# uoguelph-mlrg/Theano-MPI

Measured on NVIDIA B200. Metric: AlexNet-128b BSP seconds per 5120 images (train+comm, device-timed, max over ranks), lower is better.
Workload: dtype bf16; 1 GPU; model=AlexNet, global_batch=128, input=3x227x227, parallelism=dp1, rule=BSP, push_master=False, cuda_graph=True, overlap=True

## Files before the change

### theanompi_b200/csrc/api.h

```cpp
#pragma once
#include <cuda_runtime.h>
#include <stdint.h>
#include "common.cuh"

namespace tmpi {

constexpr int kMaxRanks = 8;
constexpr int kMaxCommBlocks = 1024;

struct CommCtx {
  void* arena[kMaxRanks];
  uint32_t* sig[kMaxRanks];
  uint32_t* epoch;
  void* mc_arena;
  int rank, world;
  long long spin_limit;
};

struct FusedArgs {
  CommCtx ctx;
  long long w_off, g_off, u_off, h_off, wire_off;
  const uint8_t* block_group;
  GroupTable tab;
  const float* lr_ptr;
  float mu;
  int nesterov;
  float inv_k;
  long long lo, hi;
  int wire16;
  int pre_reduced;
  int push_master = 1;
};

struct ReduceArgs {
  CommCtx ctx;
  long long src_off, dst_off, h_off;
  const uint8_t* block_group;
  GroupTable tab;
  float scale;
  long long lo, hi;
  int skip_local_groups;
};

void gemm_set_debug(int flags);
void gemm_set_bulk(int mask);
void gemm_rs_configure(int world, const void* const* peer_g , const void* local_g);
void gemm_rs_add_range(const void* c_lo, const void* c_hi, long long blo, long long per);
void gemm_rs_clear();
int gemm_plan_splits(int tiles, int num_kb, int sms);
int gemm_plan_tall(long long M, int nt, int out_bf16, int sms);
void gemm_bf16(const void* A, const void* B, void* C, const float* bias, int M, int N, int K, long long lda, long long ldb,
               long long ldc, int a_mn, int b_mn, int out_bf16, int bias_mode, int relu, float alpha, int bn_hint, int splitk,
               cudaStream_t st, int tf32 = 0);

void conv_fprop_bf16(const void* x, const void* w, void* y, const float* bias, int N, int H, int W, int Ctot, int c_off, int Cg, int KH,
                     int KW, int Ho, int Wo, int S, int P, int O, long long ldc, int relu, int out_bf16, int dgrad, cudaStream_t st, int tf32 = 0);
void conv_wgrad_bf16(const void* dy, const void* x, void* dw, int N, int H, int W, int Ctot, int c_off, int Cg, int KH, int KW, int Ho,
                     int Wo, int S, int P, int O, long long ldy, cudaStream_t st, int tf32 = 0);
void conv_fprop2_bf16(const void* x, const void* w0, const void* w1, void* y0, void* y1, const float* bias0, const float* bias1, int N, int H,
                      int W, int Ctot, int c_off0, int c_off1, int Cg, int KH, int KW, int Ho, int Wo, int S, int P, int O, long long ldc,
                      int relu, int out_bf16, int dgrad, cudaStream_t st, int tf32 = 0);
void conv_wgrad2_bf16(const void* dy0, const void* dy1, const void* x, void* dw0, void* dw1, int N, int H, int W, int Ctot, int c_off0,
                      int c_off1, int Cg, int KH, int KW, int Ho, int Wo, int S, int P, int O, long long ldy, cudaStream_t st, int tf32 = 0);

void space_to_depth(const void* x, void* y, int N, int H, int W, int C, int S, int Hs, int Ws, int Cp, int P, cudaStream_t st);
void s2d_filter(const void* src, void* dst, int O, int KH, int KW, int C, int S, int KHs, int KWs, int Cp, int dir, cudaStream_t st);
void conv_weight_flip(const void* w, void* wt, int O, int KH, int KW, int Cg, cudaStream_t st);
void lrn_fwd(const void* x, void* y, long long rows, int C, int n, float k, float alpha, float beta, cudaStream_t st);
void lrn_bwd(const void* x, const void* dy, void* dx, long long rows, int C, int n, float k, float alpha, float beta, cudaStream_t st);
void pool_fwd(const void* x, void* y, void* arg, int N, int H, int W, int C, int Ho, int Wo, int k, int s, int p, int is_max, cudaStream_t st);
void pool_bwd(const void* dy, const void* arg, void* dx, int N, int H, int W, int C, int Ho, int Wo, int k, int s, int p, int is_max, cudaStream_t st);
void dropout_fwd(const void* x, void* y, void* mask, long long n, float p_drop, unsigned long long seed, int layer, const void* step, cudaStream_t st);
void dropout_bwd(const void* dy, const void* mask, void* dx, long long n, cudaStream_t st);
void advance_step(void* step, cudaStream_t st);
void softmax_xent(const void* logits, const void* labels, void* dlogits, void* rowstat, void* out3, int B, int C, float weight, cudaStream_t st);
void relu_bias_bwd(const void* dy, const void* y, void* dym, void* db, long long R, int C, long long ld, int relu, cudaStream_t st);
void relu_bias_bwd2(const void* dy, const void* y, void* dym, void* db, void* db1, int c_split, long long R, int C, long long ld, int relu,
                    cudaStream_t st);
void maxpool_relu_bias_bwd(const void* dyp, const void* arg, const void* y, void* dym, void* db0, void* db1, int c_split, int N, int H,
                           int W, int C, int Ho, int Wo, int k, int s, int p, cudaStream_t st);
void im2col(const void* x, void* col, int N, int H, int W, int Ctot, int c_off, int Cg, int KH, int KW, int Ho, int Wo, int s, int p,
            long long ldcol, cudaStream_t st);
void col2im(const void* dcol, void* dx, int N, int H, int W, int Ctot, int c_off, int Cg, int KH, int KW, int Ho, int Wo, int s, int p,
            long long ldcol, cudaStream_t st);
void pad_rows(const void* src, void* dst, long long rows, int cols, long long src_ld, long long dst_ld, cudaStream_t st);
void transpose_bf16(const void* src, void* dst, int R, int C, cudaStream_t st);
// ... 8 lines not shown
void dropout_fwd_f32(const void* x, void* y, void* mask, long long n, float p_drop, unsigned long long seed, int layer, const void* step,
                     cudaStream_t st);
void dropout_bwd_f32(const void* dy, const void* mask, void* dx, long long n, cudaStream_t st);
void softmax_xent_f32(const void* logits, const void* labels, void* dlogits, void* rowstat, void* out3, int B, int C, float weight, cudaStream_t st);
void relu_bias_bwd2_f32(const void* dy, const void* y, void* dym, void* db, void* db1, int c_split, long long R, int C, long long ld, int relu,
                        cudaStream_t st);
void bias_act_f32(const void* acc, const void* bias, void* y, int R, int C, int relu, cudaStream_t st);
void im2col_f32(const void* x, void* col, int N, int H, int W, int Ctot, int c_off, int Cg, int KH, int KW, int Ho, int Wo, int s, int p,
                long long ldcol, cudaStream_t st);
void col2im_f32(const void* dcol, void* dx, int N, int H, int W, int Ctot, int c_off, int Cg, int KH, int KW, int Ho, int Wo, int s, int p,
                long long ldcol, cudaStream_t st);
void pad_rows_f32(const void* src, void* dst, long long rows, int cols, long long src_ld, long long dst_ld, cudaStream_t st);
void space_to_depth_f32(const void* x, void* y, int N, int H, int W, int C, int S, int Hs, int Ws, int Cp, int P, cudaStream_t st);
void s2d_filter_pack_f32(const void* src, void* dst, int O, int KH, int KW, int C, int S, int KHs, int KWs, int Cp, cudaStream_t st);

void bn_forward(const void* x, const void* res, void* y, const void* gamma, const void* beta, void* mean, void* rstd, void* run_mean,
                void* run_var, void* scratch, long long R, int C, float momentum, float eps, int training, int relu, int f32, cudaStream_t st);
void bn_backward(const void* x, const void* dy, const void* y, void* dx, void* dres, const void* gamma, const void* mean, const void* rstd,
                 void* dgamma, void* dbeta, void* scratch, long long R, int C, int relu, int f32, cudaStream_t st);
void add_tensors(const void* a, const void* b, void* y, long long n, int f32, cudaStream_t st);
void add4_tensors(const void* a, const void* b, const void* c, const void* d, void* y, long long n, int f32, cudaStream_t st);

void lstm_cell_fwd(const void* gx, const void* gh, const void* c_prev, const void* h_prev, const void* mask, void* act, void* c_out, void* h_out,
                   int B, int H, int f32, cudaStream_t st);
void lstm_cell_bwd(const void* dh_out, const void* dh_rec, const void* dh_pass_in, const void* dc_next, const void* act, const void* c,
                   const void* c_prev, const void* mask, void* dG, void* dc_prev, void* dh_pass, int B, int H, int f32, cudaStream_t st);
void embedding_fwd(const void* ids, const void* W, void* out, long long n, int D, int f32, cudaStream_t st);
void embedding_bwd(const void* ids, const void* dout, void* dW, long long n, int D, long long V, int f32, cudaStream_t st);
void masked_mean_fwd(const void* h, const void* mask, void* out, int Tn, int B, int H, int f32, cudaStream_t st);
void masked_mean_bwd(const void* dout, const void* mask, void* dh, int Tn, int B, int H, int f32, cudaStream_t st);

void sgd_flat(void* W, const void* G, void* U, void* H, const void* block_group, const GroupTable& tab, const void* lr_ptr, float mu,
              int nesterov, float inv_k, long long lo, long long hi, int filter, cudaStream_t st);
void adam_flat(void* W, const void* G, void* M, void* V, void* H, const void* block_group, const GroupTable& tab, const void* lr_ptr, void* step,
               float b1, float b2, float eps, long long lo, long long hi, cudaStream_t st);
void fused_allreduce_sgd(const FusedArgs& a, int algo, int max_blocks, cudaStream_t st);
void push_master_slices(const FusedArgs& a, int max_blocks, cudaStream_t st);
void allreduce_flat(const ReduceArgs& a, int algo, int max_blocks, cudaStream_t st);
void device_barrier(const CommCtx& c, cudaStream_t st);
void easgd_elastic(void* w, void* h, void* center, float alpha, long long n, int max_blocks, int lockfree, cudaStream_t st);
void ticket_acquire(const CommCtx& c, int owner, void* local_state, cudaStream_t st);
void ticket_release(const CommCtx& c, int owner, void* local_state, cudaStream_t st);
void copy_flat(void* dst, void* dst_h, const void* src, long long n, int max_blocks, const void* gate, cudaStream_t st);
void gosgd_push(const CommCtx& c, void* state, int dest, long long w_off, long long snap_off, long long n, int max_blocks, cudaStream_t st);
void gosgd_poll_merge(const CommCtx& c, void* state, long long w_off, long long h_off, long long snap_off, long long n, int max_blocks,
                      cudaStream_t st);
void gosgd_merge(void* w, void* h, const void* b, float a_self, float a_src, long long n, int max_blocks, cudaStream_t st);
void bias_act_cast(const void* acc, const void* bias, void* y, int R, int C, int relu, cudaStream_t st);
void cast_flat(const void* src, void* dst, long long n, int kind, cudaStream_t st);
void sum_chunks(const void* src, void* dst, long long chunk, int nchunks, int is_half, cudaStream_t st);
void vecadd(void* cur, const void* tmp, long long n, int is_half, cudaStream_t st);

}
```

### theanompi_b200/csrc/binding.cpp

```cpp
#include <pybind11/pybind11.h>
#include <pybind11/stl.h>

#include <cstring>
#include <memory>
#include <vector>

#include "api.h"
#include "peer_arena.h"

namespace py = pybind11;
using namespace tmpi;
typedef uintptr_t ptr_t;

static inline void* P(ptr_t p) { return reinterpret_cast<void*>(p); }
static inline cudaStream_t S(ptr_t s) { return reinterpret_cast<cudaStream_t>(s); }
static inline cudaStream_t S_(ptr_t s) { return reinterpret_cast<cudaStream_t>(s); }

static GroupTable make_table(const std::vector<float>& lr_mult, const std::vector<float>& wd, const std::vector<int>& exch) {
  GroupTable t;
  for (int i = 0; i < kMaxGroups; ++i) {
    t.lr_mult[i] = i < (int)lr_mult.size() ? lr_mult[i] : 1.f;
    t.wd[i] = i < (int)wd.size() ? wd[i] : 0.f;
    t.exch[i] = i < (int)exch.size() ? exch[i] : 1;
  }
// ... 120 lines not shown
  m.def("pad_rows_f32", [](ptr_t src, ptr_t dst, long long rows, int cols, long long src_ld, long long dst_ld, ptr_t st) {
    pad_rows_f32(P(src), P(dst), rows, cols, src_ld, dst_ld, S(st)); });
  m.def("space_to_depth_f32", [](ptr_t x, ptr_t y, int N, int H, int W, int C, int S, int Hs, int Ws, int Cp, int Pd, ptr_t st) {
    space_to_depth_f32(P(x), P(y), N, H, W, C, S, Hs, Ws, Cp, Pd, S_(st)); });
  m.def("s2d_filter_pack_f32", [](ptr_t src, ptr_t dst, int O, int KH, int KW, int C, int S, int KHs, int KWs, int Cp, ptr_t st) {
    s2d_filter_pack_f32(P(src), P(dst), O, KH, KW, C, S, KHs, KWs, Cp, S_(st)); });

  m.def("bn_forward", [](ptr_t x, ptr_t res, ptr_t y, ptr_t gamma, ptr_t beta, ptr_t mean, ptr_t rstd, ptr_t run_mean, ptr_t run_var, ptr_t scratch,
                         long long R, int C, float momentum, float eps, int training, int relu, int f32, ptr_t st) {
    bn_forward(P(x), P(res), P(y), P(gamma), P(beta), P(mean), P(rstd), P(run_mean), P(run_var), P(scratch), R, C, momentum, eps, training, relu,
               f32, S(st)); });
  m.def("bn_backward", [](ptr_t x, ptr_t dy, ptr_t y, ptr_t dx, ptr_t dres, ptr_t gamma, ptr_t mean, ptr_t rstd, ptr_t dgamma, ptr_t dbeta,
                          ptr_t scratch, long long R, int C, int relu, int f32, ptr_t st) {
    bn_backward(P(x), P(dy), P(y), P(dx), P(dres), P(gamma), P(mean), P(rstd), P(dgamma), P(dbeta), P(scratch), R, C, relu, f32, S(st)); });
  m.def("add4_tensors", [](ptr_t a, ptr_t b, ptr_t c, ptr_t d, ptr_t y, long long n, int f32, ptr_t st) {
    add4_tensors(P(a), P(b), P(c), P(d), P(y), n, f32, S(st)); });
  m.def("add_tensors", [](ptr_t a, ptr_t b, ptr_t y, long long n, int f32, ptr_t st) { add_tensors(P(a), P(b), P(y), n, f32, S(st)); });

  m.def("lstm_cell_fwd", [](ptr_t gx, ptr_t gh, ptr_t c_prev, ptr_t h_prev, ptr_t mask, ptr_t act, ptr_t c_out, ptr_t h_out, int B, int H, int f32,
                            ptr_t st) { lstm_cell_fwd(P(gx), P(gh), P(c_prev), P(h_prev), P(mask), P(act), P(c_out), P(h_out), B, H, f32, S(st)); });
  m.def("lstm_cell_bwd", [](ptr_t dh_out, ptr_t dh_rec, ptr_t dh_pass_in, ptr_t dc_next, ptr_t act, ptr_t c, ptr_t c_prev, ptr_t mask, ptr_t dG,
                            ptr_t dc_prev, ptr_t dh_pass, int B, int H, int f32, ptr_t st) {
    lstm_cell_bwd(P(dh_out), P(dh_rec), P(dh_pass_in), P(dc_next), P(act), P(c), P(c_prev), P(mask), P(dG), P(dc_prev), P(dh_pass), B, H, f32, S(st)); });
  m.def("embedding_fwd", [](ptr_t ids, ptr_t W, ptr_t out, long long n, int D, int f32, ptr_t st) { embedding_fwd(P(ids), P(W), P(out), n, D, f32, S(st)); });
  m.def("embedding_bwd", [](ptr_t ids, ptr_t dout, ptr_t dW, long long n, int D, long long V, int f32, ptr_t st) {
    embedding_bwd(P(ids), P(dout), P(dW), n, D, V, f32, S(st)); });
  m.def("masked_mean_fwd", [](ptr_t h, ptr_t mask, ptr_t out, int Tn, int B, int H, int f32, ptr_t st) { masked_mean_fwd(P(h), P(mask), P(out), Tn, B, H, f32, S(st)); });
  m.def("masked_mean_bwd", [](ptr_t dout, ptr_t mask, ptr_t dh, int Tn, int B, int H, int f32, ptr_t st) { masked_mean_bwd(P(dout), P(mask), P(dh), Tn, B, H, f32, S(st)); });

  m.def("sgd_flat", [](ptr_t W, ptr_t G, ptr_t U, ptr_t H, ptr_t block_group, std::vector<float> lr_mult, std::vector<float> wd,
                       std::vector<int> exch, ptr_t lr_ptr, float mu, int nesterov, float inv_k, long long lo, long long hi, int filter,
                       ptr_t st) {
    sgd_flat(P(W), P(G), P(U), P(H), P(block_group), make_table(lr_mult, wd, exch), P(lr_ptr), mu, nesterov, inv_k, lo, hi, filter, S(st)); });
  m.def("adam_flat", [](ptr_t W, ptr_t G, ptr_t M, ptr_t V, ptr_t H, ptr_t block_group, std::vector<float> lr_mult, std::vector<float> wd,
                        std::vector<int> exch, ptr_t lr_ptr, ptr_t step, float b1, float b2, float eps, long long lo, long long hi, ptr_t st) {
    adam_flat(P(W), P(G), P(M), P(V), P(H), P(block_group), make_table(lr_mult, wd, exch), P(lr_ptr), P(step), b1, b2, eps, lo, hi, S(st)); });
  m.def("easgd_elastic", [](ptr_t w, ptr_t h, ptr_t center, float alpha, long long n, int max_blocks, ptr_t st, int lockfree) {
    easgd_elastic(P(w), P(h), P(center), alpha, n, max_blocks, lockfree, S(st)); },
    py::arg("w"), py::arg("h"), py::arg("center"), py::arg("alpha"), py::arg("n"), py::arg("max_blocks"), py::arg("st"), py::arg("lockfree") = 0);
  m.def("copy_flat", [](ptr_t dst, ptr_t dst_h, ptr_t src, long long n, int max_blocks, ptr_t st) {
    copy_flat(P(dst), P(dst_h), P(src), n, max_blocks, nullptr, S(st)); });
  m.def("gosgd_merge", [](ptr_t w, ptr_t h, ptr_t b, float a_self, float a_src, long long n, int max_blocks, ptr_t st) {
    gosgd_merge(P(w), P(h), P(b), a_self, a_src, n, max_blocks, S(st)); });
  m.def("bias_act_cast", [](ptr_t acc, ptr_t bias, ptr_t y, int R, int C, int relu, ptr_t st) { bias_act_cast(P(acc), P(bias), P(y), R, C, relu, S(st)); });
  m.def("cast_flat", [](ptr_t src, ptr_t dst, long long n, int kind, ptr_t st) { cast_flat(P(src), P(dst), n, kind, S(st)); });
  m.def("sum_chunks", [](ptr_t src, ptr_t dst, long long chunk, int nchunks, int is_half, ptr_t st) {
    sum_chunks(P(src), P(dst), chunk, nchunks, is_half, S(st)); });
  m.def("vecadd", [](ptr_t cur, ptr_t tmp, long long n, int is_half, ptr_t st) { vecadd(P(cur), P(tmp), n, is_half, S(st)); });

  py::class_<PyComm, std::shared_ptr<PyComm>>(m, "PeerArena")
      .def(py::init([](int rank, int world, int device, unsigned long long bytes, const std::string& job, bool force_ipc) {
        auto c = std::make_shared<PyComm>();
        c->pa.reset(new PeerArena(rank, world, device, (size_t)bytes, job, force_ipc));
        return c;
      }), py::arg("rank"), py::arg("world"), py::arg("device"), py::arg("bytes"), py::arg("job"), py::arg("force_ipc") = false)
      .def("send_handles_to", [](PyComm& c, int peer) { py::gil_scoped_release r; c.pa->send_handles_to(peer); })
      .def("recv_handles", [](PyComm& c) { py::gil_scoped_release r; c.pa->recv_handles(); })
      .def("ipc_handles", [](PyComm& c) { return py::bytes(c.pa->ipc_handles()); })
      .def("ipc_open", [](PyComm& c, int peer, const std::string& h) { c.pa->ipc_open(peer, h); })
      .def("multicast_supported", [](PyComm& c) { return c.pa->multicast_supported(); })
      .def("mc_create_and_send", [](PyComm& c) { py::gil_scoped_release r; c.pa->mc_create_and_send(); })
      .def("mc_recv", [](PyComm& c) { py::gil_scoped_release r; c.pa->mc_recv(); })
      .def("mc_add_device", [](PyComm& c) { c.pa->mc_add_device(); })
      .def("mc_bind_and_map", [](PyComm& c) { c.pa->mc_bind_and_map(); })
      .def("arena_ptr", [](PyComm& c, int p) { return (ptr_t)c.pa->arena_ptr(p); })
      .def("sig_ptr", [](PyComm& c, int p) { return (ptr_t)c.pa->sig_ptr(p); })
// ... 60 lines not shown
```

### theanompi_b200/csrc/comm_kernels.cu

```cuda
#include "common.cuh"
#include "api.h"

namespace tmpi {

constexpr int kThreads = 256;

__device__ __forceinline__ float4 ld_sys_f4(const float* p) {
  float4 v;
  asm volatile("ld.volatile.global.v4.f32 {%0, %1, %2, %3}, [%4];" : "=f"(v.x), "=f"(v.y), "=f"(v.z), "=f"(v.w) : "l"(p) : "memory");
  return v;
}
__device__ __forceinline__ uint2 ld_sys_u2(const void* p) {
  uint2 v;
  asm volatile("ld.volatile.global.v2.u32 {%0, %1}, [%2];" : "=r"(v.x), "=r"(v.y) : "l"(p) : "memory");
  return v;
}
__device__ __forceinline__ void st_f4(float* p, float4 v) {
  asm volatile("st.global.v4.f32 [%0], {%1, %2, %3, %4};" ::"l"(p), "f"(v.x), "f"(v.y), "f"(v.z), "f"(v.w) : "memory");
}
__device__ __forceinline__ void st_u2(void* p, uint2 v) {
  asm volatile("st.global.v2.u32 [%0], {%1, %2};" ::"l"(p), "r"(v.x), "r"(v.y) : "memory");
}
__device__ __forceinline__ float4 mc_ld_reduce_f4(const float* mc) {
  float4 v;
// ... 58 lines not shown
  }
  TMPI_SGD1(w.x, u.x, gsum.x) TMPI_SGD1(w.y, u.y, gsum.y) TMPI_SGD1(w.z, u.z, gsum.z) TMPI_SGD1(w.w, u.w, gsum.w)
#undef TMPI_SGD1
}

__global__ void __launch_bounds__(kThreads) sgd_flat_kernel(float* __restrict__ W, const float* __restrict__ G, float* __restrict__ U,
                                                            __nv_bfloat16* __restrict__ H, const uint8_t* __restrict__ block_group,
                                                            GroupTable tab, const float* __restrict__ lr_ptr, float mu, int nesterov,
                                                            float inv_k, long long blk_lo, long long blk_hi, int filter) {
  const Hyper h{*lr_ptr, mu, inv_k, nesterov};
  for (long long b = blk_lo + blockIdx.x; b < blk_hi; b += gridDim.x) {
    const int g = block_group[b];
    if ((filter == 1 && tab.exch[g]) || (filter == 2 && !tab.exch[g])) continue;
    const long long i = b * kArenaBlock + threadIdx.x * 4;
    float4 w = *reinterpret_cast<const float4*>(W + i);
    float4 u = *reinterpret_cast<const float4*>(U + i);
    const float4 gg = *reinterpret_cast<const float4*>(G + i);
    sgd4(w, u, gg, h, tab.lr_mult[g], tab.wd[g]);
    *reinterpret_cast<float4*>(W + i) = w;
    *reinterpret_cast<float4*>(U + i) = u;
    if (H) *reinterpret_cast<uint2*>(H + i) = pack_bf16x4(w);
  }
}

void sgd_flat(void* W, const void* G, void* U, void* H, const void* block_group, const GroupTable& tab, const void* lr_ptr, float mu,
              int nesterov, float inv_k, long long lo, long long hi, int filter, cudaStream_t st) {
  if (lo % kArenaBlock || hi % kArenaBlock) throw std::runtime_error("sgd_flat: range must be block aligned");
  const long long nb = (hi - lo) / kArenaBlock;
  if (nb <= 0) return;
  int grid = (int)std::min<long long>(nb, (long long)sm_count() * 8);
  sgd_flat_kernel<<<grid, kThreads, 0, st>>>((float*)W, (const float*)G, (float*)U, (__nv_bfloat16*)H, (const uint8_t*)block_group, tab,
                                             (const float*)lr_ptr, mu, nesterov, inv_k, lo / kArenaBlock, hi / kArenaBlock, filter);
  count_launch(); TMPI_CHECK_LAUNCH("sgd_flat"); ::tmpi::check_capture(st, "sgd_flat");
}

__global__ void __launch_bounds__(kThreads) adam_flat_kernel(float* __restrict__ W, const float* __restrict__ G, float* __restrict__ M,
                                                             float* __restrict__ V, __nv_bfloat16* __restrict__ H,
                                                             const uint8_t* __restrict__ block_group, GroupTable tab,
                                                             const float* __restrict__ lr_ptr, const unsigned long long* __restrict__ step,
                                                             float b1, float b2, float eps, long long blk_lo, long long blk_hi) {
  const float t = (float)(*step + 1ull);
  const float c1 = 1.f / (1.f - __powf(b1, t)), c2 = 1.f / (1.f - __powf(b2, t));
  const float lr0 = *lr_ptr;
  for (long long b = blk_lo + blockIdx.x; b < blk_hi; b += gridDim.x) {
    const int g = block_group[b];
    const float lr = lr0 * tab.lr_mult[g], wd = tab.wd[g];
    const long long i = b * kArenaBlock + threadIdx.x * 4;
    float4 w = *reinterpret_cast<const float4*>(W + i), m = *reinterpret_cast<const float4*>(M + i), v = *reinterpret_cast<const float4*>(V + i);
    const float4 gg = *reinterpret_cast<const float4*>(G + i);
#define TMPI_ADAM1(Wc, Mc, Vc, Gc)                                    \
  {                                                                  \
    const float ge = Gc + wd * Wc;                                   \
    Mc = b1 * Mc + (1.f - b1) * ge;                                  \
    Vc = b2 * Vc + (1.f - b2) * ge * ge;                             \
    Wc -= lr * (Mc * c1) / (sqrtf(Vc * c2) + eps);                   \
  }
    TMPI_ADAM1(w.x, m.x, v.x, gg.x) TMPI_ADAM1(w.y, m.y, v.y, gg.y) TMPI_ADAM1(w.z, m.z, v.z, gg.z) TMPI_ADAM1(w.w, m.w, v.w, gg.w)
#undef TMPI_ADAM1
    *reinterpret_cast<float4*>(W + i) = w;
    *reinterpret_cast<float4*>(M + i) = m;
    *reinterpret_cast<float4*>(V + i) = v;
    if (H) *reinterpret_cast<uint2*>(H + i) = pack_bf16x4(w);
  }
}
__global__ void adam_advance_kernel(unsigned long long* step) { if (threadIdx.x == 0 && blockIdx.x == 0) *step += 1ull; }

// ... 589 lines not shown
```

### theanompi_b200/csrc/gemm_tcgen05.cu

```cuda
#include "common.cuh"
#include "api.h"
#include <cuda.h>
#include <algorithm>
#include <map>
#include <vector>
#include <mutex>
#include <tuple>

namespace tmpi {
std::atomic<unsigned long long> g_launch_count{0};

namespace gemm {

constexpr int BM = 128;
constexpr int NUM_THREADS = 320;
constexpr int NUM_EPI_WARPS = 8;

template <typename T> struct Elem {
  static constexpr int ESZ = (int)sizeof(T);
  static constexpr int BK = 128 / ESZ;
  static constexpr int UMMA_K = 32 / ESZ;
  static constexpr int ATOM = 128 / ESZ;
  static constexpr bool TF32 = ESZ == 4;
};
// ... 724 lines not shown
      for (int q = 0; q < kMaxRanks; ++q) p.rs_g[q] = q < g_rs_world ? g_rs_peer[q] : nullptr;
      return true;
    }
  }
  return false;
}
}

void gemm_rs_configure(int world, const void* const* peer_g, const void* local_g) {
  std::lock_guard<std::mutex> lk(gemm::g_rs_mu);
  if (world > kMaxRanks) throw std::runtime_error("gemm_rs_configure: too many ranks");
  gemm::g_rs_world = world;
  gemm::g_rs_local = reinterpret_cast<const char*>(local_g);
  gemm::g_rs_rank = 0;
  for (int q = 0; q < world; ++q) {
    gemm::g_rs_peer[q] = reinterpret_cast<float*>(const_cast<void*>(peer_g[q]));
    if (peer_g[q] == local_g) gemm::g_rs_rank = q;
  }
  gemm::g_rs_ranges.clear();
}
void gemm_rs_add_range(const void* c_lo, const void* c_hi, long long blo, long long per) {
  std::lock_guard<std::mutex> lk(gemm::g_rs_mu);
  gemm::g_rs_ranges.push_back({reinterpret_cast<const char*>(c_lo), reinterpret_cast<const char*>(c_hi), blo, per});
}
void gemm_rs_clear() {
  std::lock_guard<std::mutex> lk(gemm::g_rs_mu);
  gemm::g_rs_world = 0; gemm::g_rs_ranges.clear();
}

int gemm_plan_splits(int tiles, int num_kb, int sms) { return gemm::choose_splits(tiles, num_kb, sms); }
int gemm_plan_tall(long long M, int nt, int out_bf16, int sms) { return gemm::use_tall_tiles(M, nt, out_bf16, sms) ? 1 : 0; }

namespace gemm {
template <typename T>
static void gemm_host(const void* A, const void* B, void* C, const float* bias, int M, int N, int K, long long lda, long long ldb,
                      long long ldc, int a_mn, int b_mn, int out_bf16, int bias_mode, int relu, float alpha, int bn_hint, int splitk,
                      cudaStream_t st) {
  using E = Elem<T>;
  constexpr int BK = E::BK, ATOM = E::ATOM, ESZ = E::ESZ;
  if (M <= 0 || N <= 0 || K <= 0) return;
  const int sms = sm_count();
  const int mt = (M + BM - 1) / BM;
  const bool fused_epi = bias_mode != 0 || relu;
  const bool can_split = (!out_bf16) && !fused_epi;
  int BN = bn_hint;
  if (BN == 0) {
    BN = 128;
    if (!(can_split && splitk != 1)) {
      if (mt * ((N + 127) / 128) < sms && N >= 64) BN = 64;
      if (BN == 64 && mt * ((N + 63) / 64) < sms && !b_mn && N >= 32) BN = 32;
    } else if (N <= 64) {
      BN = 64;
    }
  }
  if (b_mn && BN < 64) BN = 64;
  const int nt = (N + BN - 1) / BN;
  const int num_kb = (K + BK - 1) / BK;
  int splits = 1;
  if (splitk > 1 && can_split) splits = splitk;
  else if (splitk == 0 && can_split) splits = choose_splits(mt * nt, num_kb, sms);
  int kb_per = (num_kb + splits - 1) / splits;
  splits = (num_kb + kb_per - 1) / kb_per;

  Params p;
  p.C = C; p.bias = bias; p.alpha = alpha; p.M = M; p.N = N; p.K = K; p.ldc = ldc; p.a_mn = a_mn; p.b_mn = b_mn;
  p.out_bf16 = out_bf16; p.bias_mode = bias ? bias_mode : 0; p.relu = relu; p.kb_per_split = kb_per; p.atomic_out = splits > 1;
// ... 198 lines not shown
```

### theanompi_b200/models/base.py

```python
from __future__ import annotations

import time

import numpy as np
import torch

from .. import ops
from ..parallel.arena import FlatArena
from ..utils import nvtx
from ..utils.opt import FlatSGD, SharedScalar, pre_model_iter_fn
from .layers2 import BatchNormal, Crop, Dropout, count_params


def pick_device(config):
    dev = config.get("device")
    if dev is not None:
        return torch.device(dev)
    if torch.cuda.is_available():
        return torch.device("cuda", torch.cuda.current_device())
    return torch.device("cpu")


class ModelBase(object):
    n_epochs = 1
# ... 21 lines not shown
        self.verbose = config.get("verbose", False)
        self.rank = config.get("rank", 0)
        self.size = config.get("size", 1)
        self.no_paraload = config.get("no_paraload", False)
        self.device = pick_device(config)
        self.cuda = self.device.type == "cuda"
        from ..ops import precision
        if config.get("dtype"):
            precision.set_precision(config["dtype"])
        self.precision = precision.precision()
        self.act_dtype = precision.act_dtype() if self.cuda else torch.float32
        cg = config.get("cuda_graph", "auto")
        self._graph_auto = (cg == "auto")
        if self._graph_auto and not getattr(self, "graph_safe", True):
            cg = False
        self.use_graph = bool(cg) and self.cuda
        self.epoch = 0
        self.step_idx = 0
        self.mu = self.momentum
        self.eta = self.weight_decay
        self.base_lr = np.float32(self.learning_rate)
        self.current_t = self.subb_t = 0
        self.current_v = self.subb_v = 0
        self.last_one_t = self.last_one_v = False
        self.compiled_train_fn_list = []
        self.train_iter_fn = None
        self.val_iter_fn = None
        self._graph = None
        self._graph_out = None
        self._gstream = None
        self._warm = 0
        self._tail = None
        self.exchanger = None
        self.h2d_bytes_last = 0

    def setup_data_parallel(self, data):
        self.data = data
        data.batch_data(self.file_batch_size)
        data.extend_data(rank=self.rank, size=self.size)
        data.shuffle_data(mode="train", common_seed=1234)
        data.shuffle_data(mode="val")
        data.shard_data(mode="train", rank=self.rank, size=self.size)
        data.shard_data(mode="val", rank=self.rank, size=self.size)
        self.n_subb = max(1, self.file_batch_size // self.batch_size)

    def finalize(self, params, weight_types, input_shape):
        self.params, self.weight_types = list(params), list(weight_types)
        count_params(self.params, verbose=False)
        allocator = self.config.get("arena_allocator")
        self.arena = FlatArena(self.params, self.weight_types, self.device, weight_decay=self.eta, bias_lr_mult=self.bias_lr_mult,
                               with_recv=allocator is not None, allocator=allocator,
                               shadow=False if self.precision == "tf32" else self.config.get("_arena_shadow"))
        self.shared_lr = SharedScalar(self.arena.hyper, 0, self.base_lr)
        self.sgd = FlatSGD(self.arena, self.mu, self.use_nesterov_momentum, self.use_momentum)
        B = self.batch_size
        fb = self.file_batch_size
        self.input_shape = tuple(input_shape)
        self.shared_x = torch.zeros((fb,) + self.input_shape[1:], dtype=self.act_dtype, device=self.device)
        self.shared_y = torch.zeros((fb,), dtype=torch.int64, device=self.device)
        self.x_in = torch.zeros((B,) + self.input_shape[1:], dtype=self.act_dtype, device=self.device)
        self.y_in = torch.zeros((B,), dtype=torch.int64, device=self.device)
        self._y_ring = [torch.zeros((fb,), dtype=torch.int64, pin_memory=self.cuda) for _ in range(4 if self.cuda else 1)]
        self._y_ev = [None] * len(self._y_ring)
        self._y_k = 0
        self.vels, self.vels2 = [], []
        if self.verbose:
# ... 26 lines not shown
        else:
            self.x_in.copy_(self.shared_x[subb_ind * B:(subb_ind + 1) * B], non_blocking=True)
            self.y_in.copy_(self.shared_y[subb_ind * B:(subb_ind + 1) * B], non_blocking=True)
        if not self.use_graph:
            return self._step_body()
        if self._graph is None:
            if self._gstream is None:
                self._gstream = torch.cuda.Stream(device=self.device)
            if self._warm < 2:
                self._warm += 1
                cur = torch.cuda.current_stream(self.device)
                self._gstream.wait_stream(cur)
                with torch.cuda.stream(self._gstream):
                    out = self._step_body()
                cur.wait_stream(self._gstream)
                return out
            ok, why = True, ""
            try:
                self._capture()
            except Exception as e:
                if not self._graph_auto:
                    raise
                ok, why = False, "%s: %s" % (type(e).__name__, str(e)[:200])
            ex = self.exchanger
            if ex is not None and getattr(ex, "fused", False) and getattr(ex, "size", 1) > 1:
                ok = all(ex.comm.allgather(bool(ok)))
            if not ok:
                print("[%s] CUDA-graph capture of the training step failed (%s) — running eager"
                      % (getattr(self, "name", type(self).__name__), why or "on another rank"))
                self.use_graph = False
                self._graph = None
                if ex is not None and hasattr(ex, "_reset_pending") and getattr(ex, "fused", False):
                    ex._reset_pending()
                torch.cuda.synchronize()
                return self._step_body()
        self._graph.replay()
        return self._graph_out

    def _step_body(self):
        out = self._fwd_bwd_eager()
        self._dbg_capture("forward+backward")
        if self._tail is not None:
            with torch.no_grad():
                self._tail()
            self._dbg_capture("step tail")
        self._after_step()
        return out

    def _dbg_capture(self, where):
        import os
        if not self.cuda or os.environ.get("TMPI_DEBUG_CAPTURE") != "1":
            return
        from ..ops import native
        err, status = native.require().capture_status(torch.cuda.current_stream(self.device).cuda_stream)
        if err != 0 or status == 2:
            raise RuntimeError("CUDA graph capture invalidated during %s (err %d status %d)" % (where, err, status))

    def _after_step(self):
        if self.cuda:
            from ..ops import cuda_impl
            cuda_impl.advance_step(self.device)
        else:
            ops.advance_rng_step()

    def _capture(self):
        torch.cuda.synchronize()
# ... 177 lines not shown
```

### theanompi_b200/ops/cuda_impl.py

```python
from __future__ import annotations

import os

import torch

from . import native, precision

_STEP = {}
BF16 = torch.bfloat16
F32 = torch.float32


def ADT():
    return precision.act_dtype()


def _is32(t):
    return t.dtype == F32


def _al(t):
    return 16 // t.element_size()


# ... 541 lines not shown
    mode = 0 if mean.numel() == 1 else (1 if mean.numel() == C else 2)
    if mode == 2:
        assert mean.numel() == H * W * C
    Cout = c_out or C
    if out is None:
        out = torch.empty((N, ch, cw, Cout), dtype=out_dtype, device=x.device)
    assert out.dtype in (BF16, torch.float32)
    offsets = offsets.to(torch.int32).contiguous()
    flips = flips.to(torch.uint8).contiguous()
    if isinstance(std_scale, torch.Tensor):
        cs = std_scale.to(device=x.device, dtype=torch.float32).contiguous()
        assert cs.numel() == C
        sc, cs_ptr = 1.0, cs.data_ptr()
    else:
        sc, cs_ptr = float(std_scale), 0
    L().crop_mirror_norm(x.data_ptr(), kind, mean.data_ptr(), mode, sc, cs_ptr, out.data_ptr(), int(out.dtype == BF16),
                         offsets.data_ptr(), flips.data_ptr(), N, H, W, C, ch, cw, Cout, _st(x))
    return out


def _table(arena):
    if not hasattr(arena, "_tab_cache"):
        arena._tab_cache = (arena.group_lr_mult_np.tolist(), arena.group_wd_np.tolist(),
                            [int(v) for v in arena.group_exch_np.tolist()])
    return arena._tab_cache


def sgd_flat(arena, g, lr, mu, nesterov, inv_k, lo, hi, only_local=False, only_exchanged=False):
    lrm, wd, ex = _table(arena)
    filt = 1 if only_local else (2 if only_exchanged else 0)
    H = arena.H
    L().sgd_flat(arena.W.data_ptr(), g.data_ptr(), arena.U.data_ptr(), _p(H), arena.block_group.data_ptr(), lrm, wd, ex,
                 arena.hyper.data_ptr(), float(mu), int(bool(nesterov)), float(inv_k), int(lo), int(hi), filt, _st(arena.W))
```

### theanompi_b200/utils/opt.py

```python
from __future__ import annotations

import torch

from ..ops import reference as ref


class SharedScalar(object):

    def __init__(self, buf, index, value=0.0):
        self._buf, self._i = buf, index
        self._host = float(value)
        self.set_value(value)

    def get_value(self):
        return self._host

    def set_value(self, v):
        self._host = float(v)
        self._buf[self._i] = float(v)


def _native_for(t):
    if t.is_cuda:
        from ..ops import cuda_impl
# ... 6 lines not shown
    def __init__(self, arena, mu=0.9, nesterov=False, use_momentum=True):
        self.arena = arena
        self.mu = mu if use_momentum else 0.0
        self.nesterov = nesterov

    def step(self, lr, k=1, src="G", lo=0, hi=None, only_local=False, only_exchanged=False):
        a = self.arena
        hi = a.numel if hi is None else hi
        g = getattr(a, src)
        nat = _native_for(a.W)
        if nat is not None:
            nat.sgd_flat(a, g, lr, self.mu, self.nesterov, 1.0 / k, lo, hi,
                         only_local=only_local, only_exchanged=only_exchanged)
            return
        sl = slice(lo, hi)
        lrm, wd = a.lr_mult_vector()[sl], a.wd_vector()[sl]
        w, gg, u = a.W[sl], g[sl], a.U[sl]
        if only_local or only_exchanged:
            ex = a.exch_vector()[sl]
            m = ~ex if only_local else ex
            idx = m.nonzero().squeeze(1)
            if idx.numel() == 0:
                return
            w2, u2 = w[idx].clone(), u[idx].clone()
            ref.sgd_flat(w2, gg[idx], u2, lrm[idx], wd[idx], lr, self.mu, self.nesterov, 1.0 / k)
            w[idx] = w2
            u[idx] = u2
        else:
            ref.sgd_flat(w, gg, u, lrm, wd, lr, self.mu, self.nesterov, 1.0 / k)
        if a.H is not None:
            a.H[sl].copy_(w)


class FlatAdam(object):

    def __init__(self, arena, b1=0.9, b2=0.999, eps=1e-8):
        self.arena, self.b1, self.b2, self.eps = arena, b1, b2, eps
        self.V = torch.zeros_like(arena.W)
        self.t = torch.zeros(1, dtype=torch.int64, device=arena.W.device)

    def step(self, lr=None):
        a = self.arena
        nat = _native_for(a.W)
        if nat is not None:
            from ..ops.cuda_impl import L, _table, _p, _st
            lrm, wd, ex = _table(a)
            L().adam_flat(a.W.data_ptr(), a.G.data_ptr(), a.U.data_ptr(), self.V.data_ptr(), _p(a.H), a.block_group.data_ptr(), lrm, wd, ex,
                          a.hyper.data_ptr(), self.t.data_ptr(), float(self.b1), float(self.b2), float(self.eps), 0, int(a.numel), _st(a.W))
            return
        lr = float(a.hyper[0]) if lr is None else lr
        self.t += 1
        t = float(self.t)
        g = a.G + a.wd_vector() * a.W
        a.U.mul_(self.b1).add_(g, alpha=1 - self.b1)
        self.V.mul_(self.b2).addcmul_(g, g, value=1 - self.b2)
        mh, vh = a.U / (1 - self.b1 ** t), self.V / (1 - self.b2 ** t)
        a.W.sub_(lr * a.lr_mult_vector() * mh / (vh.sqrt() + self.eps))
        if a.H is not None:
            a.H.copy_(a.W)

    def state_dict(self):
        return {"V": self.V.detach().cpu(), "t": int(self.t)}

    def load_state_dict(self, sd):
        self.V.copy_(sd["V"].to(self.V.device)); self.t.fill_(int(sd["t"]))

# ... 91 lines not shown


def BSP_MSGD(model, use_nesterov_momentum, k=1):
    return _publish(model, *_pre_post_msgd(model, use_nesterov_momentum, k), k)


def _BSP_MSGD(model, use_nesterov_momentum, k=1):
    return _publish(model, *_pre_post_msgd_grad(model, use_nesterov_momentum, k), k)


def BSP_SGD(model, k=1):
    return _publish(model, *_pre_post_sgd(model, k), k)


def _clip_paramlist(param_list, scale=10):
    with torch.no_grad():
        for p in param_list:
            p.clamp_(-scale, scale)
    return param_list


def prepare_update_dict(model, k=1, aggregate="momentum"):
    if model.use_momentum:
        if aggregate == "gradient":
            return _BSP_MSGD(model, model.use_nesterov_momentum, k=k)
        return BSP_MSGD(model, model.use_nesterov_momentum, k=k)
    return BSP_SGD(model, k=k)


def pre_model_iter_fn(model, k=1, f_train=True, f_val=True, aggregate="momentum", fused_tail=None):
    if f_train:
        pre, post = prepare_update_dict(model, k=k, aggregate=aggregate)
        tail = fused_tail if fused_tail is not None else (pre if k == 1 else None)
        model.set_step_tail(tail)

        def get_vel(subb_ind=0):
            cost, err = model.forward_backward(subb_ind)
            if tail is None:
                with torch.no_grad():
                    pre()
            return cost, err

        def descent_vel():
            if tail is None:
                with torch.no_grad():
                    post()

        model.get_vel, model.descent_vel = get_vel, descent_vel
        model.compiled_train_fn_list = [get_vel, descent_vel]
        model.train_iter_fn = choose_iter_fn(model)
    if f_val:
        model.compile_val()
        model.val_iter_fn = model.val_fn


def choose_iter_fn(model):

    def cdd_iter_fn(subb_ind=0):
        return model.get_vel(subb_ind)

    return cdd_iter_fn
```

Before: 0.06600 s/5120img.

## Overlap bucketed local SGD updates with backward pass on a side stream

For the single-worker k=1 case, a BucketedSGD object splits the parameter arena into buckets and launches an SGD update kernel for each bucket on a side stream once all of its parameters' gradients are ready. The aim is to hide the optimizer tail behind the remaining backward compute. A new unrolled, register-capped SGD kernel with optional streaming cache hints is added, along with function-attribute introspection bindings. The update kernels now compete with backward kernels for SMs, and correctness depends on the on_ready hooks firing and on the pending counts being reset when the CUDA graph is recaptured.

```diff
diff --git a/theanompi_b200/csrc/api.h b/theanompi_b200/csrc/api.h
--- a/theanompi_b200/csrc/api.h
+++ b/theanompi_b200/csrc/api.h
@@ -1,6 +1,9 @@
 #pragma once
 #include <cuda_runtime.h>
 #include <stdint.h>
+#include <string>
+#include <utility>
+#include <vector>
 #include "common.cuh"
 
 namespace tmpi {
@@ -32,6 +35,10 @@
   int push_master = 1;
 };
 
+struct FuncAttrs {
+  int num_regs, max_threads, static_smem, dyn_smem, local_bytes;
+};
+
 struct ReduceArgs {
   CommCtx ctx;
   long long src_off, dst_off, h_off;
@@ -52,6 +59,7 @@
 void gemm_bf16(const void* A, const void* B, void* C, const float* bias, int M, int N, int K, long long lda, long long ldb,
                long long ldc, int a_mn, int b_mn, int out_bf16, int bias_mode, int relu, float alpha, int bn_hint, int splitk,
                cudaStream_t st, int tf32 = 0);
+void gemm_func_attrs(std::vector<std::pair<std::string, FuncAttrs>>& out);
 
 void conv_fprop_bf16(const void* x, const void* w, void* y, const float* bias, int N, int H, int W, int Ctot, int c_off, int Cg, int KH,
                      int KW, int Ho, int Wo, int S, int P, int O, long long ldc, int relu, int out_bf16, int dgrad, cudaStream_t st, int tf32 = 0);
@@ -126,6 +134,10 @@
 
 void sgd_flat(void* W, const void* G, void* U, void* H, const void* block_group, const GroupTable& tab, const void* lr_ptr, float mu,
               int nesterov, float inv_k, long long lo, long long hi, int filter, cudaStream_t st);
+void sgd_flat_overlap(void* W, const void* G, void* U, void* H, const void* block_group, const GroupTable& tab, const void* lr_ptr,
+                      float mu, int nesterov, float inv_k, long long lo, long long hi, int filter, int unroll, int max_blocks,
+                      int streaming, cudaStream_t st);
+void comm_func_attrs(std::vector<std::pair<std::string, FuncAttrs>>& out);
 void adam_flat(void* W, const void* G, void* M, void* V, void* H, const void* block_group, const GroupTable& tab, const void* lr_ptr, void* step,
                float b1, float b2, float eps, long long lo, long long hi, cudaStream_t st);
 void fused_allreduce_sgd(const FusedArgs& a, int algo, int max_blocks, cudaStream_t st);
diff --git a/theanompi_b200/csrc/binding.cpp b/theanompi_b200/csrc/binding.cpp
--- a/theanompi_b200/csrc/binding.cpp
+++ b/theanompi_b200/csrc/binding.cpp
@@ -176,6 +176,24 @@
                        std::vector<int> exch, ptr_t lr_ptr, float mu, int nesterov, float inv_k, long long lo, long long hi, int filter,
                        ptr_t st) {
     sgd_flat(P(W), P(G), P(U), P(H), P(block_group), make_table(lr_mult, wd, exch), P(lr_ptr), mu, nesterov, inv_k, lo, hi, filter, S(st)); });
+  m.def("sgd_flat_overlap", [](ptr_t W, ptr_t G, ptr_t U, ptr_t H, ptr_t block_group, std::vector<float> lr_mult, std::vector<float> wd,
+                               std::vector<int> exch, ptr_t lr_ptr, float mu, int nesterov, float inv_k, long long lo, long long hi, int filter,
+                               int unroll, int max_blocks, int streaming, ptr_t st) {
+    sgd_flat_overlap(P(W), P(G), P(U), P(H), P(block_group), make_table(lr_mult, wd, exch), P(lr_ptr), mu, nesterov, inv_k, lo, hi, filter,
+                     unroll, max_blocks, streaming, S(st)); });
+  m.def("func_attrs", [] {
+    std::vector<std::pair<std::string, FuncAttrs>> v;
+    gemm_func_attrs(v);
+    comm_func_attrs(v);
+    py::dict d;
+    for (const auto& kv : v) {
+      py::dict a;
+      a["num_regs"] = kv.second.num_regs; a["max_threads"] = kv.second.max_threads; a["static_smem"] = kv.second.static_smem;
+      a["dyn_smem"] = kv.second.dyn_smem; a["local_bytes"] = kv.second.local_bytes;
+      d[py::str(kv.first)] = a;
+    }
+    return d;
+  });
   m.def("adam_flat", [](ptr_t W, ptr_t G, ptr_t M, ptr_t V, ptr_t H, ptr_t block_group, std::vector<float> lr_mult, std::vector<float> wd,
                         std::vector<int> exch, ptr_t lr_ptr, ptr_t step, float b1, float b2, float eps, long long lo, long long hi, ptr_t st) {
     adam_flat(P(W), P(G), P(M), P(V), P(H), P(block_group), make_table(lr_mult, wd, exch), P(lr_ptr), P(step), b1, b2, eps, lo, hi, S(st)); });
diff --git a/theanompi_b200/csrc/comm_kernels.cu b/theanompi_b200/csrc/comm_kernels.cu
--- a/theanompi_b200/csrc/comm_kernels.cu
+++ b/theanompi_b200/csrc/comm_kernels.cu
@@ -114,6 +114,95 @@
   sgd_flat_kernel<<<grid, kThreads, 0, st>>>((float*)W, (const float*)G, (float*)U, (__nv_bfloat16*)H, (const uint8_t*)block_group, tab,
                                              (const float*)lr_ptr, mu, nesterov, inv_k, lo / kArenaBlock, hi / kArenaBlock, filter);
   count_launch(); TMPI_CHECK_LAUNCH("sgd_flat"); ::tmpi::check_capture(st, "sgd_flat");
+}
+
+template <bool CS> __device__ __forceinline__ float4 ld_f4(const float* p) {
+  return CS ? __ldcs(reinterpret_cast<const float4*>(p)) : *reinterpret_cast<const float4*>(p);
+}
+template <bool CS> __device__ __forceinline__ void st_f4_hint(float* p, float4 v) {
+  if (CS) __stcs(reinterpret_cast<float4*>(p), v); else *reinterpret_cast<float4*>(p) = v;
+}
+template <bool CS> __device__ __forceinline__ void st_u2_hint(__nv_bfloat16* p, uint2 v) {
+  if (CS) __stcs(reinterpret_cast<uint2*>(p), v); else *reinterpret_cast<uint2*>(p) = v;
+}
+
+constexpr int kOverlapMaxRegs = 96;
+
+template <int U_, bool CS>
+__global__ void __maxnreg__(kOverlapMaxRegs)
+sgd_flat_overlap_kernel(float* __restrict__ W, const float* __restrict__ G, float* __restrict__ U, __nv_bfloat16* __restrict__ H,
+                        const uint8_t* __restrict__ block_group, GroupTable tab, const float* __restrict__ lr_ptr, float mu, int nesterov,
+                        float inv_k, long long blk_lo, long long blk_hi, int filter) {
+  const Hyper h{*lr_ptr, mu, inv_k, nesterov};
+  for (long long b0 = blk_lo + blockIdx.x; b0 < blk_hi; b0 += (long long)gridDim.x * U_) {
+    float4 w[U_], u[U_], g[U_];
+    int grp[U_];
+#pragma unroll
+    for (int k = 0; k < U_; ++k) {
+      const long long b = b0 + (long long)k * gridDim.x;
+      grp[k] = -1;
+      if (b < blk_hi) {
+        const long long i = b * kArenaBlock + threadIdx.x * 4;
+        grp[k] = block_group[b];
+        w[k] = ld_f4<CS>(W + i);
+        u[k] = ld_f4<CS>(U + i);
+        g[k] = ld_f4<CS>(G + i);
+      }
+    }
+#pragma unroll
+    for (int k = 0; k < U_; ++k) {
+      const int gi = grp[k];
+      if (gi < 0 || (filter == 1 && tab.exch[gi]) || (filter == 2 && !tab.exch[gi])) continue;
+      const long long i = (b0 + (long long)k * gridDim.x) * kArenaBlock + threadIdx.x * 4;
+      sgd4(w[k], u[k], g[k], h, tab.lr_mult[gi], tab.wd[gi]);
+      st_f4_hint<CS>(W + i, w[k]);
+      st_f4_hint<CS>(U + i, u[k]);
+      if (H) st_u2_hint<CS>(H + i, pack_bf16x4(w[k]));
+    }
+  }
+}
+
+template <int U_, bool CS> static void launch_sgd_overlap(int grid, cudaStream_t st, void* W, const void* G, void* U, void* H,
+                                                          const void* block_group, const GroupTable& tab, const void* lr_ptr, float mu,
+                                                          int nesterov, float inv_k, long long blo, long long bhi, int filter) {
+  sgd_flat_overlap_kernel<U_, CS><<<grid, kThreads, 0, st>>>((float*)W, (const float*)G, (float*)U, (__nv_bfloat16*)H,
+                                                             (const uint8_t*)block_group, tab, (const float*)lr_ptr, mu, nesterov, inv_k,
+                                                             blo, bhi, filter);
+}
+
+void sgd_flat_overlap(void* W, const void* G, void* U, void* H, const void* block_group, const GroupTable& tab, const void* lr_ptr,
+                      float mu, int nesterov, float inv_k, long long lo, long long hi, int filter, int unroll, int max_blocks,
+                      int streaming, cudaStream_t st) {
+  if (lo % kArenaBlock || hi % kArenaBlock) throw std::runtime_error("sgd_flat_overlap: range must be block aligned");
+  if (unroll != 2 && unroll != 4) throw std::runtime_error("sgd_flat_overlap: unroll must be 2 or 4");
+  const long long nb = (hi - lo) / kArenaBlock;
+  if (nb <= 0) return;
+  long long cap = sm_count();
+  if (max_blocks > 0) cap = std::min<long long>(cap, max_blocks);
+  const int grid = (int)std::min<long long>(nb, cap);
+  const long long blo = lo / kArenaBlock, bhi = hi / kArenaBlock;
+  if (unroll == 2) {
+    if (streaming) launch_sgd_overlap<2, true>(grid, st, W, G, U, H, block_group, tab, lr_ptr, mu, nesterov, inv_k, blo, bhi, filter);
+    else launch_sgd_overlap<2, false>(grid, st, W, G, U, H, block_group, tab, lr_ptr, mu, nesterov, inv_k, blo, bhi, filter);
+  } else {
+    if (streaming) launch_sgd_overlap<4, true>(grid, st, W, G, U, H, block_group, tab, lr_ptr, mu, nesterov, inv_k, blo, bhi, filter);
+    else launch_sgd_overlap<4, false>(grid, st, W, G, U, H, block_group, tab, lr_ptr, mu, nesterov, inv_k, blo, bhi, filter);
+  }
+  count_launch(); TMPI_CHECK_LAUNCH("sgd_flat_overlap"); ::tmpi::check_capture(st, "sgd_flat_overlap");
+}
+
+static FuncAttrs attrs_of(const void* fn, int dyn_smem) {
+  cudaFuncAttributes a;
+  check_cuda(cudaFuncGetAttributes(&a, fn), "cudaFuncGetAttributes");
+  return FuncAttrs{a.numRegs, a.maxThreadsPerBlock, (int)a.sharedSizeBytes, dyn_smem, (int)a.localSizeBytes};
+}
+
+void comm_func_attrs(std::vector<std::pair<std::string, FuncAttrs>>& out) {
+  out.emplace_back("sgd_flat", attrs_of((const void*)sgd_flat_kernel, 0));
+  out.emplace_back("sgd_flat_overlap_u2", attrs_of((const void*)sgd_flat_overlap_kernel<2, false>, 0));
+  out.emplace_back("sgd_flat_overlap_u2_cs", attrs_of((const void*)sgd_flat_overlap_kernel<2, true>, 0));
+  out.emplace_back("sgd_flat_overlap_u4", attrs_of((const void*)sgd_flat_overlap_kernel<4, false>, 0));
+  out.emplace_back("sgd_flat_overlap_u4_cs", attrs_of((const void*)sgd_flat_overlap_kernel<4, true>, 0));
 }
 
 __global__ void __launch_bounds__(kThreads) adam_flat_kernel(float* __restrict__ W, const float* __restrict__ G, float* __restrict__ M,
diff --git a/theanompi_b200/csrc/gemm_tcgen05.cu b/theanompi_b200/csrc/gemm_tcgen05.cu
--- a/theanompi_b200/csrc/gemm_tcgen05.cu
+++ b/theanompi_b200/csrc/gemm_tcgen05.cu
@@ -780,6 +780,23 @@
 int gemm_plan_tall(long long M, int nt, int out_bf16, int sms) { return gemm::use_tall_tiles(M, nt, out_bf16, sms) ? 1 : 0; }
 
 namespace gemm {
+template <typename T, int BN, int MT> static void add_attrs(std::vector<std::pair<std::string, FuncAttrs>>& out) {
+  cudaFuncAttributes a;
+  check_cuda(cudaFuncGetAttributes(&a, (const void*)gemm_tcgen05<T, BN, MT>), "cudaFuncGetAttributes");
+  const std::string name = std::string(sizeof(T) == 4 ? "gemm_tf32_" : "gemm_bf16_") + std::to_string(BN) + "x" + std::to_string(MT);
+  out.emplace_back(name, FuncAttrs{a.numRegs, a.maxThreadsPerBlock, (int)a.sharedSizeBytes, Cfg<T, BN, MT>::SMEM_BYTES, (int)a.localSizeBytes});
+}
+template <typename T> static void add_attrs_all(std::vector<std::pair<std::string, FuncAttrs>>& out) {
+  add_attrs<T, 128, 1>(out); add_attrs<T, 64, 1>(out); add_attrs<T, 32, 1>(out); add_attrs<T, 128, 2>(out); add_attrs<T, 64, 2>(out);
+}
+}
+
+void gemm_func_attrs(std::vector<std::pair<std::string, FuncAttrs>>& out) {
+  gemm::add_attrs_all<__nv_bfloat16>(out);
+  gemm::add_attrs_all<float>(out);
+}
+
+namespace gemm {
 template <typename T>
 static void gemm_host(const void* A, const void* B, void* C, const float* bias, int M, int N, int K, long long lda, long long ldb,
                       long long ldc, int a_mn, int b_mn, int out_bf16, int bias_mode, int relu, float alpha, int bn_hint, int splitk,
diff --git a/theanompi_b200/models/base.py b/theanompi_b200/models/base.py
--- a/theanompi_b200/models/base.py
+++ b/theanompi_b200/models/base.py
@@ -77,6 +77,7 @@
         self._warm = 0
         self._tail = None
         self.exchanger = None
+        self.local_overlap = None
         self.h2d_bytes_last = 0
 
     def setup_data_parallel(self, data):
@@ -169,6 +170,8 @@
                 self._graph = None
                 if ex is not None and hasattr(ex, "_reset_pending") and getattr(ex, "fused", False):
                     ex._reset_pending()
+                if getattr(self, "local_overlap", None) is not None:
+                    self.local_overlap.reset()
                 torch.cuda.synchronize()
                 return self._step_body()
         self._graph.replay()
diff --git a/theanompi_b200/ops/cuda_impl.py b/theanompi_b200/ops/cuda_impl.py
--- a/theanompi_b200/ops/cuda_impl.py
+++ b/theanompi_b200/ops/cuda_impl.py
@@ -597,3 +597,10 @@
     H = arena.H
     L().sgd_flat(arena.W.data_ptr(), g.data_ptr(), arena.U.data_ptr(), _p(H), arena.block_group.data_ptr(), lrm, wd, ex,
                  arena.hyper.data_ptr(), float(mu), int(bool(nesterov)), float(inv_k), int(lo), int(hi), filt, _st(arena.W))
+
+
+def sgd_flat_overlap(arena, mu, nesterov, lo, hi, unroll=4, max_blocks=0, streaming=False):
+    lrm, wd, ex = _table(arena)
+    L().sgd_flat_overlap(arena.W.data_ptr(), arena.G.data_ptr(), arena.U.data_ptr(), _p(arena.H), arena.block_group.data_ptr(), lrm, wd,
+                         ex, arena.hyper.data_ptr(), float(mu), int(bool(nesterov)), 1.0, int(lo), int(hi), 0, int(unroll),
+                         int(max_blocks), int(bool(streaming)), _st(arena.W))
diff --git a/theanompi_b200/utils/opt.py b/theanompi_b200/utils/opt.py
--- a/theanompi_b200/utils/opt.py
+++ b/theanompi_b200/utils/opt.py
@@ -62,6 +62,63 @@
             a.H[sl].copy_(w)
 
 
+class BucketedSGD(object):
+
+    BUCKET_BYTES = 32 << 20
+    TAIL_BYTES = 4 << 20
+
+    def __init__(self, arena, mu, nesterov):
+        import os
+        self.arena, self.mu, self.nesterov = arena, mu, nesterov
+        self.unroll = int(os.environ.get("TMPI_LOCAL_SGD_UNROLL", "4"))
+        self.max_blocks = int(os.environ.get("TMPI_LOCAL_SGD_BLOCKS", "0"))
+        self.streaming = os.environ.get("TMPI_LOCAL_SGD_CS", "0") == "1"
+        self.buckets = arena.make_buckets(self.BUCKET_BYTES, tail_bytes=self.TAIL_BYTES)
+        self._bucket_of = {}
+        for bi, b in enumerate(self.buckets):
+            for pi in b["params"]:
+                self._bucket_of[id(arena.params[pi])] = bi
+        self.side = torch.cuda.Stream(device=arena.device) if arena.device.type == "cuda" else None
+        self._pending = [0] * len(self.buckets)
+        self.reset()
+        for p in arena.params:
+            p.on_ready = self._on_ready
+
+    def detach(self):
+        for p in self.arena.params:
+            if getattr(p, "on_ready", None) == self._on_ready:
+                p.on_ready = None
+
+    def reset(self):
+        for bi, b in enumerate(self.buckets):
+            self._pending[bi] = len(b["params"])
+        self._launched = 0
+
+    def _launch(self, bi):
+        from ..ops import cuda_impl
+        b = self.buckets[bi]
+        self.side.wait_stream(torch.cuda.current_stream(self.arena.device))
+        with torch.cuda.stream(self.side):
+            cuda_impl.sgd_flat_overlap(self.arena, self.mu, self.nesterov, b["lo"], b["hi"], self.unroll, self.max_blocks, self.streaming)
+
+    def _launch_ready(self):
+        while self._launched < len(self.buckets) and self._pending[self._launched] <= 0:
+            self._launch(self._launched)
+            self._launched += 1
+
+    def _on_ready(self, p):
+        self._pending[self._bucket_of[id(p)]] -= 1
+        self._launch_ready()
+
+    def step(self):
+        for bi in range(self._launched, len(self.buckets)):
+            self._pending[bi] = 0
+        self._launch_ready()
+        if self.side is not None:
+            torch.cuda.current_stream(self.arena.device).wait_stream(self.side)
+        self.reset()
+
+
 class FlatAdam(object):
 
     def __init__(self, arena, b1=0.9, b2=0.999, eps=1e-8):
@@ -219,6 +276,16 @@
     if f_train:
         pre, post = prepare_update_dict(model, k=k, aggregate=aggregate)
         tail = fused_tail if fused_tail is not None else (pre if k == 1 else None)
+        if fused_tail is None:
+            old = getattr(model, "local_overlap", None)
+            if old is not None:
+                old.detach()
+            model.local_overlap = None
+            if k == 1 and model.arena.W.is_cuda and model.config.get("overlap", True):
+                mu = model.mu if model.use_momentum else 0.0
+                nesterov = model.use_nesterov_momentum and model.use_momentum
+                model.local_overlap = BucketedSGD(model.arena, mu, nesterov)
+                tail = model.local_overlap.step
         model.set_step_tail(tail)
 
         def get_vel(subb_ind=0):
```

After: 0.06469 s/5120img, median of 6. 2.0% less time.
